# harshadms/galileo-sdr-sim

Hardware: AMD Instinct MI355X
Metric: IQ Msamples/s (×real-time @2.6MS/s), 12-SV static E1B/C, 1/2/4/8 GPU (higher is better)
Workload: dtype f64 (NCO phases) + int16x2 (packed accumulate) -> int16 IQ; 1 GPU; M-SYN12: static-geometry 12-SV E1B/C, 1199 epochs x 260000 samples @2.6 MS/s per GPU (one independent scenario per rank); channels=12, chunk_samples=1024, walk_passes=1, synth_runs_max=1, chain_mismatch=0, pipeline_depth=2, window_mode=1, kernel_family=1, output_checksum=26e91314

## Files before the change

### galileo-sdr-sim_amd/csrc/synth_group.hip

```cpp
#include <hip/hip_runtime.h>
#include <stdint.h>
#include <type_traits>

#include "nco_walk.h"
#include "synth_dev.h"
#include "synth_common.h"

using namespace galnco;
using namespace galdev;

#if !defined(GAL_GTU)
#define GAL_GTU_MAIN 1
#define GAL_GTU_WIDE 1
#define GAL_GTU_SEARCH 1
#else
#define GAL_GTU_MAIN (GAL_GTU == 0)
#define GAL_GTU_WIDE (GAL_GTU == 1)
#define GAL_GTU_SEARCH (GAL_GTU == 2)
#endif

#ifndef SG_THREADS
#define SG_THREADS 1024
#endif
#ifndef SG_WAVES_PER_EU
#define SG_WAVES_PER_EU 4
#endif
#define SG_CHUNK 1024
#define SG_SYMS 64
#define SG_STR_PITCH 580
#define SG_MPOS 17
#define SG_LUT_N 1152
#define SG_AMB 128u
#define SG_BIAS (1049088.0 + 1.4901161193847656250e-08)
#define SG_MAXCH 12
#define SG_MAXCH_WIDE 24

struct SgRec {
    double yc;
    double pm;
    double s;
    double dabs;
};
typedef uint32_t sg_u4 __attribute__((ext_vector_type(4)));
typedef const __attribute__((address_space(3))) sg_u4 *sg_lds_u4;
typedef const __attribute__((address_space(3))) int *sg_lds_int;
typedef const __attribute__((address_space(3))) uint32_t *sg_lds_u32;

__device__ __forceinline__ uint32_t sg_rep(const uint32_t w, const int d)
{
    const uint32_t lo = (uint32_t)__builtin_amdgcn_sbfe((int)w, 2 * d, 1);
    const uint32_t hi = (uint32_t)__builtin_amdgcn_sbfe((int)w, 2 * d + 1, 1);
    return gal_bfi(0x55555555u, lo, hi);
}

__device__ __forceinline__ double sg_f64(const uint32_t lo, const uint32_t hi) { return u2d(((uint64_t)hi << 32) | lo); }

template <int J0, int CNT, int MODE, int SIG, int BINS, int BPITCH, bool SEARCH>
__device__ __forceinline__ void sg_part(int (&o)[16], uint32_t &amb, uint64_t &undec, const double g16, const SgRec *rec, const uint32_t *sya,
                                        const double *s_c511, const uint32_t *s_lutd,
                                        const uint32_t *s_str, const uint2 *s_bin, const uint4 *s_pat, const uint2 *s_bin6,
                                        const uint32_t *s_pat6, const float *s_thr, const int nact)
{
    uint32_t X[CNT];
    [[maybe_unused]] uint32_t XB[CNT];
    double t[CNT];
    double c511[CNT];
    uint32_t lutd[CNT];
#pragma unroll
    for (int q = 0; q < CNT; ++q) {
        c511[q] = ((const volatile __attribute__((address_space(3))) double *)(uintptr_t)s_c511)[J0 + q];
        lutd[q] = ((const volatile __attribute__((address_space(3))) uint32_t *)(uintptr_t)s_lutd)[J0 + q];
    }
    {
        int ic0[CNT];
        float f[CNT];
        uint2 be[CNT];
        uint32_t lo[CNT], hi[CNT], mask[CNT];
        double praw[CNT];
        [[maybe_unused]] float f6[CNT];
        [[maybe_unused]] uint2 be6[CNT];
        [[maybe_unused]] int i12[CNT];
#pragma unroll
        for (int q = 0; q < CNT; ++q) {
            const int j = J0 + q;
            const sg_u4 r0 = ((sg_lds_u4)(uintptr_t)(rec + j))[0], r1 = ((sg_lds_u4)(uintptr_t)(rec + j))[1];
            const uint32_t sa0 = *(sg_lds_u32)(uintptr_t)(sya + j);
            const double A = __builtin_fma(g16, sg_f64(r1.x, r1.y), sg_f64(r0.x, r0.y));
            ic0[q] = (int)A;
            f[q] = (float)__builtin_amdgcn_fract(A);
            if constexpr (!SEARCH) {
                const int bi = (int)(f[q] * (float)BINS);
                be[q] = s_bin[j * BPITCH + bi];
            }
            if constexpr (SIG == 1) {
                const double y6 = 6.0 * A;
                i12[q] = (int)y6;
                f6[q] = (float)__builtin_amdgcn_fract(y6);
                be6[q] = s_bin6[j * CB_BIN_PITCH + (int)(f6[q] * (float)CB_BINS)];
            }
            const uint32_t *wp = s_str + j * SG_STR_PITCH + (ic0[q] >> 4);
            lo[q] = wp[0];
            hi[q] = wp[1];
            int pos;
            asm("v_med3_i32 %0, %1, 0, 16" : "=v"(pos) : "v"(ic0[q] - (8184 - 16)));
            mask[q] = *(sg_lds_u32)(uintptr_t)(sa0 + ((uint32_t)pos << 2));
            praw[q] = __builtin_fma(g16, sg_f64(r1.z, r1.w), sg_f64(r0.z, r0.w));
        }
        uint4 M[CNT];
        [[maybe_unused]] uint32_t p6[CNT];
#pragma unroll
        for (int q = 0; q < CNT; ++q) {
            const int j = J0 + q;
            if constexpr (SIG == 1) {
                const float thr6 = __uint_as_float(be6[q].x);
                const uint32_t po6 = be6[q].y + (f6[q] >= thr6 ? 4u : 0u);
                p6[q] = *reinterpret_cast<const uint32_t *>(reinterpret_cast<const char *>(s_pat6 + j * 16) + po6) ^
                        (((uint32_t)i12[q] & 1u) ? 0xAAAAAAAAu : 0u);
                undec |= __builtin_amdgcn_ballot_w64(!(__builtin_fabsf(f6[q] - thr6) >= RW_DELTA));
            }
            if constexpr (SEARCH) {
                const float *th = s_thr + j * 16;
                int id = th[7] <= f[q] ? 8 : 0;
                id += th[id + 3] <= f[q] ? 4 : 0;
                id += th[id + 1] <= f[q] ? 2 : 0;
                id += th[id] <= f[q] ? 1 : 0;
                const float up = th[id], lo = th[id > 0 ? id - 1 : 0];
                M[q] = s_pat[j * 16 + id];
                const bool near = !(up - f[q] >= RW_DELTA) | ((id > 0) & !(f[q] - lo >= RW_DELTA)) | !(f[q] >= RW_DELTA) | !(f[q] <= 1.0f - RW_DELTA);
                undec |= __builtin_amdgcn_ballot_w64(near);
            } else {
            const float thr = __uint_as_float(be[q].x);
            const uint32_t po = be[q].y + (f[q] >= thr ? 16u : 0u);
            M[q] = *reinterpret_cast<const uint4 *>(reinterpret_cast<const char *>(s_pat + j * 16) + po);
            undec |= __builtin_amdgcn_ballot_w64(!(__builtin_fabsf(f[q] - thr) >= RW_DELTA));
            }
            const double pg = praw[q] - __builtin_trunc(praw[q]);
            t[q] = __builtin_fma(511.0, pg, SG_BIAS);
        }
#pragma unroll
        for (int q = 0; q < CNT; ++q) {
            const uint32_t W = __builtin_amdgcn_alignbit(hi[q], lo[q], (uint32_t)ic0[q] << 1) ^ mask[q];
            if constexpr (SIG == 1) {
                uint32_t x, hw;
                if constexpr (MODE == 1) {
                    x = rw_spread(W, M[q]);
                    hw = ((M[q].x ^ M[q].y ^ M[q].z ^ M[q].w) & 0xAAAAAAAAu) ^ 0x22222222u;
                } else if constexpr (MODE == 4) {
                    x = gal_bfi(M[q].w, W << 16, W);
                    x = gal_bfi(M[q].z, x << 8, x);
                    x = gal_bfi(M[q].y, x << 4, x);
                    x = gal_bfi(M[q].x, x << 2, x);
                    hw = (M[q].x & 0xAAAAAAAAu) ^ 0x22222222u;
                } else {
                    x = gal_bfi(M[q].x, sg_rep(W, 1), sg_rep(W, 0));
                    x = gal_bfi(M[q].y, sg_rep(W, 2), x);
                    if constexpr (MODE == 3) {
                        x = gal_bfi(M[q].z, sg_rep(W, 3), x);
                        x = gal_bfi(M[q].w, sg_rep(W, 4), x);
                    }
                    hw = ((M[q].x ^ M[q].y ^ M[q].z ^ M[q].w) & 0xAAAAAAAAu) ^ 0xAAAAAAAAu;
                }
                hw ^= ((uint32_t)ic0[q] & 1u) ? 0xAAAAAAAAu : 0u;
                X[q] = window_signed(x);
                const uint32_t sb = x ^ hw ^ p6[q];
                const uint32_t lo1 = ~x & 0x55555555u;
                XB[q] = (J0 + q) < nact ? (lo1 | (sb & (lo1 << 1))) : 0u;
            } else if constexpr (MODE == 1) {
                X[q] = rw_spread(window_signed(W), M[q]);
            } else if constexpr (MODE == 4) {
                uint32_t x = window_signed(W);
                x = gal_bfi(M[q].w, x << 16, x);
                x = gal_bfi(M[q].z, x << 8, x);
                x = gal_bfi(M[q].y, x << 4, x);
                X[q] = gal_bfi(M[q].x, x << 2, x);
            } else {
                const uint32_t w = window_signed(W);
                uint32_t x = gal_bfi(M[q].x, sg_rep(w, 1), sg_rep(w, 0));
                x = gal_bfi(M[q].y, sg_rep(w, 2), x);
                if constexpr (MODE == 3) {
                    x = gal_bfi(M[q].z, sg_rep(w, 3), x);
                    x = gal_bfi(M[q].w, sg_rep(w, 4), x);
                }
                X[q] = x;
            }
        }
    }
    __builtin_amdgcn_sched_barrier(0);
    typedef int sg_i2 __attribute__((ext_vector_type(2)));
    typename std::conditional<SIG == 1, sg_i2, int>::type e[16][CNT];
    uint32_t lw[16][CNT];
#define SG_ISSUE(u)                                                                                                       \
    _Pragma("unroll") for (int q = 0; q < CNT; ++q) {                                                                     \
        if constexpr (SIG == 1) {                                                                                         \
            uint32_t a_;                                                                                                  \
            asm volatile("v_lshl_add_u32 %1, %2, 3, %3\n\tds_read_b64 %0, %1"                                             \
                         : "=&v"(e[u][q]), "=&v"(a_) : "v"((uint32_t)(d2u(t[q]) >> 32)), "v"(lutd[q]) : "memory");        \
        } else {                                                                                                          \
            asm volatile("v_lshl_add_u32 %0, %1, 2, %2\n\tds_read_b32 %0, %0"                                             \
                         : "=&v"(e[u][q]) : "v"((uint32_t)(d2u(t[q]) >> 32)), "v"(lutd[q]) : "memory");                   \
        }                                                                                                                 \
        lw[u][q] = (uint32_t)d2u(t[q]);                                                                                   \
        t[q] = t[q] + c511[q];                                                                                            \
    }
#define SG_WAIT(TXT, u)                                                                                                               \
    if constexpr (CNT == 1) asm volatile(TXT : "+v"(e[u][0]), "+v"(amb), "+v"(o[(u) ? (u) - 1 : 0]) :: "memory");                     \
    if constexpr (CNT == 2) asm volatile(TXT : "+v"(e[u][0]), "+v"(e[u][1]), "+v"(amb), "+v"(o[(u) ? (u) - 1 : 0]) :: "memory");      \
    if constexpr (CNT == 3) asm volatile(TXT : "+v"(e[u][0]), "+v"(e[u][1]), "+v"(e[u][2]), "+v"(amb), "+v"(o[(u) ? (u) - 1 : 0]) :: "memory"); \
    if constexpr (CNT == 4) asm volatile(TXT : "+v"(e[u][0]), "+v"(e[u][1]), "+v"(e[u][2]), "+v"(e[u][3]), "+v"(amb), "+v"(o[(u) ? (u) - 1 : 0]) :: "memory");
    SG_ISSUE(0)
#pragma unroll
    for (int u = 0; u < 16; ++u) {
        if (u < 15) {
            SG_ISSUE(u + 1)
            if constexpr (CNT == 1) { SG_WAIT("s_waitcnt lgkmcnt(1)", u) }
            if constexpr (CNT == 2) { SG_WAIT("s_waitcnt lgkmcnt(2)", u) }
            if constexpr (CNT == 3) { SG_WAIT("s_waitcnt lgkmcnt(3)", u) }
            if constexpr (CNT == 4) { SG_WAIT("s_waitcnt lgkmcnt(4)", u) }
        } else {
            SG_WAIT("s_waitcnt lgkmcnt(0)", u)
        }
        int acc = o[u];
#pragma unroll
        for (int q = 0; q < CNT; ++q) {
            if constexpr (SIG == 1) {
                gal_acc(acc, e[u][q].x, __builtin_amdgcn_sbfe((int)X[q], (uint32_t)(2 * u), 2));
                gal_acc(acc, e[u][q].y, __builtin_amdgcn_sbfe((int)XB[q], (uint32_t)(2 * u), 2));
            } else {
                gal_acc(acc, e[u][q], __builtin_amdgcn_sbfe((int)X[q], (uint32_t)(2 * u), 2));
            }
        }
#pragma unroll
        for (int q = 0; q < CNT; ++q) amb = amb < lw[u][q] ? amb : lw[u][q];
        o[u] = acc;
    }
#undef SG_WAIT
#undef SG_ISSUE
    __builtin_amdgcn_sched_barrier(0);
}

template <int NCH, bool ACC, int MODE, int SIG = 0, bool SEARCH = false>
__global__ __launch_bounds__(SG_THREADS) __attribute__((amdgpu_waves_per_eu(SG_WAVES_PER_EU)))
void k_synth_g(const DevPlan *__restrict__ Pd, SynGeom G, const uint8_t *__restrict__ act_all, const int *__restrict__ nact_all,
               uint32_t *__restrict__ iq, uint32_t *__restrict__ flist, const int flist_cap)
{
    static_assert(NCH >= 1 && NCH <= SG_MAXCH_WIDE, "1..24 channel positions per launch");
    static_assert(SIG == 0 || NCH <= SG_MAXCH, "the CBOC mode is built for up to 12 positions per launch");
    static_assert(!SEARCH || (SIG == 0 && NCH <= SG_MAXCH), "the threshold search is built for BOC(1,1), up to 12 positions per launch");
    constexpr int MC = NCH <= SG_MAXCH ? SG_MAXCH : SG_MAXCH_WIDE;
    constexpr int BINS = SIG ? CB_BINS : RW_BINS, BPITCH = SIG ? CB_BIN_PITCH : RW_BIN_PITCH;
    __shared__ uint32_t s_str[NCH * SG_STR_PITCH];
    __shared__ uint32_t s_mtab[16 * SG_MPOS];
    __shared__ __attribute__((aligned(8))) int s_lut[2 * SG_LUT_N * (SIG ? 2 : 1)];
    __shared__ uint2 s_bin[NCH * BPITCH];
    __shared__ uint4 s_pat[NCH * 16];
    __shared__ float s_thr[NCH * 16];
    __shared__ uint2 s_bin6[SIG ? NCH * CB_BIN_PITCH : 1];
    __shared__ uint32_t s_pat6[SIG ? NCH * 16 : 1];
    __shared__ float s_thr6[SIG ? NCH * 16 : 1];
    __shared__ uint32_t s_sym[NCH * SG_SYMS];
    __shared__ __attribute__((aligned(16))) SgRec s_rec[(SG_THREADS / 64) * 2 * MC];
    __shared__ double s_c511[MC];
    __shared__ uint32_t s_lutd[MC];
    __shared__ uint32_t s_sya[(SG_THREADS / 64) * 2 * MC];
    __shared__ int s_rwbad;

    const int tid = threadIdx.x;
    const int nthr = blockDim.x;
#ifdef SG_BALANCED_RANGES
    const int nb = (int)gridDim.x;
    const int xb = (nb & 7) == 0 ? (int)(blockIdx.x & 7) * (nb >> 3) + (int)(blockIdx.x >> 3) : (int)blockIdx.x;
    const long long U = (long long)G.ne * G.nchunks;
    long long uq = U * xb / nb;
    const long long u_end = U * (xb + 1) / nb;
#else
    const int bpe = G.blocks_per_epoch;
    const int er = (int)blockIdx.x / bpe, tg = (int)blockIdx.x - er * bpe;
    const int c_begin = G.nchunks * tg / bpe, c_end = G.nchunks * (tg + 1) / bpe;
#endif
    const int *const p_lut = Pd->lut;
    const int *const p_prn = Pd->prn;
    const int *const p_ib0 = Pd->ib0;
    const uint32_t *const p_str = Pd->str;
    const double *const p_cpx = Pd->cp_x, *const p_cpp = Pd->cp_p;
    const uint32_t *const p_cpi = Pd->cp_ib;
    const double *const p_cstep = Pd->cstep, *const p_dstep = Pd->dstep;
    const uint32_t *const p_pcur = Pd->page_cur, *const p_pnext = Pd->page_next;
    const uint32_t cs25 = Pd->cs25;
    int *const p_ctr = Pd->ctr;
    for (int i = tid; i < 16 * SG_MPOS; i += nthr) {
        const int pair = i / SG_MPOS, pos = i - pair * SG_MPOS;
        const uint32_t mc = (uint32_t)(pair >> 2) * 0x55555555u, mn = (uint32_t)(pair & 3) * 0x55555555u;
        s_mtab[i] = pos == 0 ? mc : pos == 16 ? mn : (mc ^ ((mc ^ mn) & (~0u << (2 * (16 - pos)))));
    }
    for (int i = tid; i < 2 * SG_LUT_N * (SIG ? 2 : 1); i += nthr) {
        if constexpr (SIG == 1) {
            const int ie = i >> 1, tab = ie >= SG_LUT_N, ii = ie - tab * SG_LUT_N;
            int k = ii < 512 ? ii - 511 : ii - 512;
            k = k >= 511 ? k - 511 : k;
            k = k >= 511 ? k - 511 : k;
            s_lut[i] = p_lut[((i & 1) << 9) + ((tab ? -k : k) & 511)];
            continue;
        }
        const int tab = i >= SG_LUT_N, ii = i - tab * SG_LUT_N;
        int k = ii < 512 ? ii - 511 : ii - 512;
        k = k >= 511 ? k - 511 : k;
        k = k >= 511 ? k - 511 : k;
        s_lut[i] = p_lut[(tab ? -k : k) & 511];
    }
#ifdef SG_BALANCED_RANGES
    int row_prn[NCH];
#pragma unroll
    for (int j = 0; j < NCH; ++j) row_prn[j] = 0;
#endif
#ifdef SG_BALANCED_RANGES
    bool first_seg = true;
    while (uq < u_end) {
    const int er = (int)(uq / G.nchunks);
    const int c_begin = (int)(uq - (long long)er * G.nchunks);
    const int c_end = (long long)(G.nchunks - c_begin) < u_end - uq ? G.nchunks : c_begin + (int)(u_end - uq);
    uq += c_end - c_begin;
    if (!first_seg) __syncthreads();
    first_seg = false;
#else
    {
#endif
    const int e = G.e0 + er;

    const int nact = __builtin_amdgcn_readfirstlane(nact_all[e]);
    const uint4 aw = *reinterpret_cast<const uint4 *>(act_all + (size_t)e * GAL_ACT_ROW);
    const uint4 aw2 = MC > 16 ? *reinterpret_cast<const uint4 *>(act_all + (size_t)e * GAL_ACT_ROW + 16) : make_uint4(0u, 0u, 0u, 0u);
    const uint32_t awv[8] = {aw.x, aw.y, aw.z, aw.w, aw2.x, aw2.y, aw2.z, aw2.w};
    int ixs[MC];
#pragma unroll
    for (int j = 0; j < MC; ++j) {
        ixs[j] = __builtin_amdgcn_readfirstlane(e * G.S + (int)((awv[j >> 2] >> (8 * (j & 3))) & 0xffu));
    }

    if (tid == 0) s_rwbad = 0;
#pragma unroll
    for (int j = 0; j < NCH; ++j) {
        int prn = __builtin_amdgcn_readfirstlane(p_prn[ixs[j]]);
        prn = prn < 1 ? 1 : prn;
        const bool on = j < nact;
#ifdef SG_BALANCED_RANGES
        const int want = on ? prn : -1;
        if (want == row_prn[j]) continue;
        row_prn[j] = want;
#endif
        const uint32_t *src = p_str + (size_t)(prn - 1) * STR_WORDS;
        for (int t = tid; t < STR_WORDS - 1; t += nthr) s_str[j * SG_STR_PITCH + t] = on ? src[t] : 0u;
        if (tid < SG_STR_PITCH - (STR_WORDS - 1)) {
            const int t = tid;
            const uint32_t w = t == 0 ? ((src[STR_WORDS - 1] & 0xffffu) | (src[0] << 16)) : ((src[t - 1] >> 16) | (src[t] << 16));
            s_str[j * SG_STR_PITCH + STR_WORDS - 1 + t] = on ? w : 0u;
        }
    }
    for (int i = tid; i < NCH * SG_SYMS; i += nthr) {
        const int j = i / SG_SYMS, k = i - j * SG_SYMS;
        int ix = 0;
#pragma unroll
        for (int q = 0; q < NCH; ++q) ix = j == q ? ixs[q] : ix;
        int ibit = p_ib0[ix] + k;
        const bool nx = ibit >= GAL_N_SYM_PAGE;
        ibit = nx ? ibit - GAL_N_SYM_PAGE : ibit;
        const uint32_t *pg = (nx ? p_pnext : p_pcur) + (size_t)ix * GAL_PAGE_WORDS;
        const uint32_t dbit = (pg[ibit >> 5] >> (ibit & 31)) & 1u;
        const uint32_t sbit = (cs25 >> (ibit % 25)) & 1u;
        const uint32_t sg = (dbit ^ sbit) | (sbit << 1);
        s_sym[i] = j < nact ? sg : 0u;
    }
    double rw_s[NCH];
#pragma unroll
    for (int j = 0; j < NCH; ++j) rw_s[j] = j < nact ? uniform_f64(2.0 * p_cstep[ixs[j]]) : 0.0;
    auto rw_step_of = [&](const int jj) {
        double v = 0.0;
#pragma unroll
        for (int j = 0; j < NCH; ++j) v = jj == j ? rw_s[j] : v;
        return v;
    };
    if (tid < MC) {
        int ix = 0;
#pragma unroll
        for (int q = 0; q < NCH; ++q) ix = tid == q ? ixs[q] : ix;
        const double d = (tid < NCH && tid < nact) ? p_dstep[ix] : 0.0;
        s_c511[tid] = 511.0 * __builtin_fabs(d);
        s_lutd[tid] = SIG ? (uint32_t)(uintptr_t)(sg_lds_int)s_lut + (((uint32_t)(d2u(d) >> 32) >> 31) ? SG_LUT_N * 8u : 0u) - (0x41300000u << 3)
                          : (uint32_t)(uintptr_t)(sg_lds_int)s_lut + (((uint32_t)(d2u(d) >> 32) >> 31) ? SG_LUT_N * 4u : 0u) - (0x41300000u << 2);
    }
    for (int t = tid; t < NCH * 16; t += nthr) {
        const int j = t >> 4, u = (t & 15) + 1;
        const double s = rw_step_of(j);
        if (u <= 15) {
            const double us = (double)u * s;
            const double T = 1.0 - (us - __builtin_floor(us));
            int rank = 0;
            for (int v = 1; v <= 15; ++v) {
                const double vs = (double)v * s;
                const double Tv = 1.0 - (vs - __builtin_floor(vs));
                rank += (Tv < T) || (Tv == T && v < u);
            }
            s_thr[j * 16 + rank] = (float)T;
        } else {
            s_thr[j * 16 + 15] = 2.0f;
        }
        if constexpr (SIG == 1) {
            const double s6 = 6.0 * s;
            if (u <= 15) {
                const double us = (double)u * s6;
                const double T = 1.0 - (us - __builtin_floor(us));
                int rank = 0;
                for (int v = 1; v <= 15; ++v) {
                    const double vs = (double)v * s6;
                    const double Tv = 1.0 - (vs - __builtin_floor(vs));
                    rank += (Tv < T) || (Tv == T && v < u);
                }
                s_thr6[j * 16 + rank] = (float)T;
            } else {
                s_thr6[j * 16 + 15] = 2.0f;
            }
        }
    }
    __syncthreads();
    auto build_bins = [&](uint2 *bins, const float *thrs, const int nbins, const int pitch, const uint32_t unit) {
        for (int t = tid; t < NCH * (nbins + 1); t += nthr) {
            const int j = t / (nbins + 1), b = t - j * (nbins + 1);
            const float lo = (float)b * (1.0f / (float)nbins) - RW_EDGE, hi = (float)(b + 1) * (1.0f / (float)nbins) + RW_EDGE;
            const float *th = thrs + j * 16;
            int idb = th[7] < lo ? 8 : 0;
            idb += th[idb + 3] < lo ? 4 : 0;
            idb += th[idb + 1] < lo ? 2 : 0;
            idb += th[idb] < lo ? 1 : 0;
            const float t0 = th[idb], t1 = idb < 15 ? th[idb + 1] : 2.0f;
            int cnt = (t0 < hi) + (t1 < hi);
            float thr = t0 < hi ? t0 : 4.0f;
            uint32_t off = (uint32_t)idb * unit;
            if (b == 0) { thr = cnt ? __builtin_nanf("") : 0.0f; off -= cnt ? 0u : unit; cnt = 0; }
            if (b == nbins - 1) { thr = cnt ? __builtin_nanf("") : 1.0f; cnt = 0; }
            if (cnt >= 2 || b == nbins) thr = __builtin_nanf("");
            if (j >= nact) { thr = 4.0f; off = 0u; }
            bins[j * pitch + b] = make_uint2(__float_as_uint(thr), off);
        }
    };
    if constexpr (!SEARCH) build_bins(s_bin, s_thr, BINS, BPITCH, 16u);
    if constexpr (SIG == 1) {
        build_bins(s_bin6, s_thr6, CB_BINS, CB_BIN_PITCH, 4u);
        for (int t = tid; t < NCH * 16; t += nthr) {
            const int j = t >> 4, id = t & 15;
            const double s6 = 6.0 * rw_step_of(j);
            const double Tlo = id ? (double)s_thr6[j * 16 + id - 1] : 0.0;
            double Thi = (double)s_thr6[j * 16 + id];
            Thi = Thi > 1.0 ? 1.0 : Thi;
            const double f = 0.5 * (Tlo + Thi);
            uint32_t w = 0u;
            for (int u = 1; u <= 15; ++u)
                if ((long long)__builtin_floor(f + (double)u * s6) & 1LL) w |= 2u << (2 * u);
            s_pat6[t] = j < nact ? w : 0u;
        }
    }
    for (int t = tid; t < NCH * 16; t += nthr) {
        const int j = t >> 4, id = t & 15;
        const double s = rw_step_of(j);
        const double Tlo = id ? (double)s_thr[j * 16 + id - 1] : 0.0;
        double Thi = (double)s_thr[j * 16 + id];
        Thi = Thi > 1.0 ? 1.0 : Thi;
        const double f = 0.5 * (Tlo + Thi);
        uint32_t m0 = 0u, m1 = 0u, m2 = 0u, m3 = 0u;
        if constexpr (MODE == 4) {
            for (int u = 0; u <= 15; ++u) {
                const int hld = u - (int)__builtin_floor(f + (double)u * s);
                int pp = u;
                m0 |= (hld & 1) ? 3u << (2 * pp) : 0u;
                pp -= hld & 1;
                m1 |= (hld & 2) ? 3u << (2 * pp) : 0u;
                pp -= hld & 2;
                m2 |= (hld & 4) ? 3u << (2 * pp) : 0u;
                pp -= hld & 4;
                m3 |= (hld & 8) ? 3u << (2 * pp) : 0u;
            }
            if (j >= nact) m0 = m1 = m2 = m3 = 0u;
        } else {
        int d = 0;
        double gp = 0.0;
        for (int u = 1; u <= 15; ++u) {
            const double g = __builtin_floor(f + (double)u * s);
            if ((MODE >= 2) ? (g != gp) : (g == gp)) {
                const uint32_t m = ~0u << (2 * u);
                m0 = d == 0 ? m : m0; m1 = d == 1 ? m : m1; m2 = d == 2 ? m : m2; m3 = d == 3 ? m : m3;
                ++d;
            }
            gp = g;
        }
        if (j >= nact) m0 = m1 = m2 = m3 = 0u;
        else if (d > (MODE == 2 ? 2 : 4)) s_rwbad = 1;
        }
        s_pat[t] = make_uint4(m0, m1, m2, m3);
    }
    __syncthreads();
    const bool rw_off = __builtin_amdgcn_readfirstlane(s_rwbad) != 0;

    const int lane = tid & 63;
    const int wv = tid >> 6;
    const int nw = nthr >> 6;
    const double g16 = (double)(16 * lane);
    const int jl = lane < NCH ? lane : NCH - 1;
    int ixl = 0;
#pragma unroll
    for (int q = 0; q < NCH; ++q) ixl = jl == q ? ixs[q] : ixl;
    const bool onl = jl < nact;
    const size_t cpl = (size_t)ixl * G.CP1;
    const double dl = onl ? p_dstep[ixl] : 0.0;
    const double sl = onl ? 2.0 * p_cstep[ixl] : 0.0, dabsl = __builtin_fabs(dl);
    const uint32_t dsgnl = (uint32_t)(d2u(dl) >> 32) & 0x80000000u;
    const uint32_t *const syml = s_sym + jl * SG_SYMS - (onl ? p_ib0[ixl] : 0);
    const uint32_t mtab0 = (uint32_t)(uintptr_t)(sg_lds_u32)s_mtab;
    SgRec *const recw = s_rec + wv * 2 * MC;
    uint32_t *const syaw = s_sya + wv * 2 * MC;
    const int cstep_w = nw;
    int c = __builtin_amdgcn_readfirstlane(c_begin + wv);
    double lx = 0.0, lp = 0.0;
    uint32_t lib = 0u;
    typedef const __attribute__((address_space(1))) double *sg_gbl_f64;
    typedef const __attribute__((address_space(1))) uint32_t *sg_gbl_u32;
    const sg_gbl_f64 g_cpx = (sg_gbl_f64)(uintptr_t)p_cpx + cpl, g_cpp = (sg_gbl_f64)(uintptr_t)p_cpp + cpl;
    const sg_gbl_u32 g_cpi = (sg_gbl_u32)(uintptr_t)p_cpi + cpl;
    auto fetch = [&](const int cc) {
        const int ce = cc < c_end ? cc : c_end - 1;
        lx = g_cpx[ce];
        lp = g_cpp[ce];
        lib = g_cpi[ce];
    };
    auto stage = [&](const int buf) {
        SgRec r;
        const bool pend = lx >= 4092.0;
        const double x = pend ? lx - 4092.0 : lx;
        r.yc = onl ? x + x : 0.5;
        r.pm = onl ? u2d(d2u(lp) ^ ((uint64_t)dsgnl << 32)) : 0.25;
        if (onl && dabsl == 0.0) {
            const int k = (int)(511.0 * r.pm);
            r.pm = ((double)(k >= 0 ? k : k - 1) + 0.5) * (1.0 / 511.0);
        }
        r.s = sl;
        r.dabs = dabsl;
        if (lane < NCH) {
            recw[buf * MC + lane] = r;
            const uint32_t ks = onl ? (lib & 0xffffu) + 500u * (lib >> 16) + (pend ? 1u : 0u) : 0u;
            const uint32_t pair = syml[ks] * 4u + syml[ks + 1];
            syaw[buf * MC + lane] = mtab0 + pair * (SG_MPOS * 4u);
        }
    };
    if (c < c_end) fetch(c);
    int buf = 0;
    for (; c < c_end; c += cstep_w, buf ^= 1) {
        stage(buf);
        fetch(c + cstep_w);
        const int n0 = c * SG_CHUNK;
        const int nsteps = G.N - n0 - 16 * lane;
        if (nsteps > 0) {
        uint32_t *out = iq + (size_t)er * G.N + n0 + 16 * lane;
        const bool vec_ok = ((((size_t)er * G.N + n0) & 3) == 0) && nsteps >= 16;
        int o[16];
        if (ACC) {
            if (vec_ok) {
#pragma unroll
                for (int q = 0; q < 4; ++q) {
                    const uint4 v = *reinterpret_cast<const uint4 *>(out + 4 * q);
                    o[4 * q] = (int)v.x; o[4 * q + 1] = (int)v.y; o[4 * q + 2] = (int)v.z; o[4 * q + 3] = (int)v.w;
                }
            } else {
#pragma unroll
                for (int u = 0; u < 16; ++u) o[u] = u < nsteps ? (int)out[u] : 0;
            }
        } else {
#pragma unroll
            for (int u = 0; u < 16; ++u) o[u] = 0;
        }
        uint32_t amb = ~0u;
        uint64_t undec = rw_off ? ~0ull : 0ull;
        const SgRec *rec = recw + buf * MC;
        const uint32_t *sya = syaw + buf * MC;
#define SG_PART(J0, CNT) sg_part<J0, CNT, MODE, SIG, BINS, BPITCH, SEARCH>(o, amb, undec, g16, rec, sya, s_c511, s_lutd, s_str, s_bin, s_pat, s_bin6, s_pat6, s_thr, nact); \
                         __builtin_amdgcn_sched_barrier(0);
        if constexpr (SIG == 1 && NCH <= 3) { SG_PART(0, NCH) }
        else if constexpr (SIG == 1 && NCH == 4) { SG_PART(0, 2) SG_PART(2, 2) }
        else if constexpr (SIG == 1 && NCH == 5) { SG_PART(0, 3) SG_PART(3, 2) }
        else if constexpr (SIG == 1 && NCH == 6) { SG_PART(0, 3) SG_PART(3, 3) }
        else if constexpr (SIG == 1 && NCH == 7) { SG_PART(0, 3) SG_PART(3, 2) SG_PART(5, 2) }
        else if constexpr (SIG == 1 && NCH == 8) { SG_PART(0, 3) SG_PART(3, 3) SG_PART(6, 2) }
        else if constexpr (SIG == 1 && NCH == 9) { SG_PART(0, 3) SG_PART(3, 3) SG_PART(6, 3) }
        else if constexpr (SIG == 1 && NCH == 10) { SG_PART(0, 3) SG_PART(3, 3) SG_PART(6, 2) SG_PART(8, 2) }
        else if constexpr (SIG == 1 && NCH == 11) { SG_PART(0, 3) SG_PART(3, 3) SG_PART(6, 3) SG_PART(9, 2) }
        else if constexpr (SIG == 1 && NCH == 12) { SG_PART(0, 3) SG_PART(3, 3) SG_PART(6, 3) SG_PART(9, 3) }
        else if constexpr (NCH <= 4) { SG_PART(0, NCH) }
        else if constexpr (NCH == 5) { SG_PART(0, 3) SG_PART(3, 2) }
        else if constexpr (NCH == 6) { SG_PART(0, 3) SG_PART(3, 3) }
        else if constexpr (NCH == 7) { SG_PART(0, 4) SG_PART(4, 3) }
        else if constexpr (NCH == 8) { SG_PART(0, 4) SG_PART(4, 4) }
        else if constexpr (NCH == 9) { SG_PART(0, 3) SG_PART(3, 3) SG_PART(6, 3) }
        else if constexpr (NCH == 10) { SG_PART(0, 4) SG_PART(4, 3) SG_PART(7, 3) }
        else if constexpr (NCH == 11) { SG_PART(0, 4) SG_PART(4, 4) SG_PART(8, 3) }
        else if constexpr (NCH == 12) { SG_PART(0, 4) SG_PART(4, 4) SG_PART(8, 4) }
        else {
            SG_PART(0, 4) SG_PART(4, 4)
            constexpr int R8 = NCH - 8;
            if constexpr (R8 == 5) { SG_PART(8, 3) SG_PART(11, 2) }
            else if constexpr (R8 == 6) { SG_PART(8, 3) SG_PART(11, 3) }
            else if constexpr (R8 == 7) { SG_PART(8, 4) SG_PART(12, 3) }
            else {
                SG_PART(8, 4)
                constexpr int R12 = NCH - 12;
                if constexpr (R12 <= 4) { SG_PART(12, R12) }
                else if constexpr (R12 == 5) { SG_PART(12, 3) SG_PART(15, 2) }
                else if constexpr (R12 == 6) { SG_PART(12, 3) SG_PART(15, 3) }
                else if constexpr (R12 == 7) { SG_PART(12, 4) SG_PART(16, 3) }
                else {
                    SG_PART(12, 4)
                    constexpr int R16 = NCH - 16;
                    if constexpr (R16 <= 4) { SG_PART(16, R16) }
                    else if constexpr (R16 == 5) { SG_PART(16, 3) SG_PART(19, 2) }
                    else if constexpr (R16 == 6) { SG_PART(16, 3) SG_PART(19, 3) }
                    else if constexpr (R16 == 7) { SG_PART(16, 4) SG_PART(20, 3) }
                    else { SG_PART(16, 4) SG_PART(20, 4) }
                }
            }
        }
#undef SG_PART
        if (vec_ok) {
#pragma unroll
            for (int q = 0; q < 4; ++q)
                *reinterpret_cast<uint4 *>(out + 4 * q) = make_uint4((uint32_t)o[4 * q], (uint32_t)o[4 * q + 1], (uint32_t)o[4 * q + 2], (uint32_t)o[4 * q + 3]);
        } else {
#pragma unroll
            for (int u = 0; u < 16; ++u)
                if (u < nsteps) out[u] = (uint32_t)o[u];
        }
        if (((undec >> lane) & 1ull) | (amb < SG_AMB)) {
            const int slot = atomicAdd(p_ctr + CTR_GFLAGS, 1);
            if (slot < flist_cap) flist[slot] = ((uint32_t)er * (uint32_t)G.nchunks + (uint32_t)c) * 64u + (uint32_t)lane;
        }
        }
    }
    }
}

#if GAL_GTU_MAIN
__global__ __launch_bounds__(256) void k_repair_g(DevPlan P, SynGeom G, uint32_t *__restrict__ iq, const uint32_t *__restrict__ flist,
                                                  const int flist_cap)
{
    __shared__ int s_lut[1024];
    const int n_raw = P.ctr[CTR_GFLAGS];
    const int n = n_raw < flist_cap ? n_raw : flist_cap;
    if (n_raw > flist_cap && blockIdx.x == 0 && threadIdx.x == 0) P.ctr[CTR_GOVER] = 1;
    const int gt = blockIdx.x * blockDim.x + threadIdx.x;
    const int r = threadIdx.x & 15;
    const int nrows = (gridDim.x * blockDim.x) >> 4;
    if (((int)blockIdx.x * (int)blockDim.x >> 4) >= n) return;
    for (int i = threadIdx.x; i < 1024; i += blockDim.x) s_lut[i] = P.lut[i];
    __syncthreads();
    for (int i = gt >> 4; i < n; i += nrows) {
        const uint32_t ent = flist[i];
        const int g = (int)(ent & 63u);
        const uint32_t ec = ent >> 6;
        const int er = (int)(ec / (uint32_t)G.nchunks), c = (int)(ec - (uint32_t)er * (uint32_t)G.nchunks);
        const int e = G.e0 + er;
        const int n0 = c * G.R + 16 * g;
        int cnt = G.N - n0;
        cnt = cnt > 16 ? 16 : cnt;
        int aI[16], aQ[16];
#pragma unroll
        for (int u = 0; u < 16; ++u) aI[u] = aQ[u] = 0;
        for (int s = r; s < G.S; s += 16) {
            const int idx = e * G.S + s;
            const int prn = P.prn[idx];
            if (prn <= 0) continue;
            const size_t cp = (size_t)idx * G.CP1 + c;
            const double cst = P.cstep[idx], d = P.dstep[idx];
            const uint32_t cib = P.cp_ib[cp];
            const CodeEnd ce = code_walk(P.cp_x[cp], (int)(cib & 0xffffu), cst, 1.0 / cst, 16 * g, 1 << 30, [](int, double, int, int) {});
            double x = ce.x;
            double p = carr_walk_track(P.cp_p[cp], d, 1.0 / __builtin_fabs(d), 16 * g, 16 * g + 1, 16 * g + 1, [](int, double) {}).p;
            {
                int nR = G.N - c * G.R;
                nR = nR > G.R ? G.R : nR;
                const int rem = nR - 16 * g;
                const CodeEnd ce2 = code_walk(ce.x, ce.ibit, cst, 1.0 / cst, rem, 1 << 30, [](int, double, int, int) {});
                const uint32_t fl_end = (cib >> 16) | (uint32_t)ce.flipped | (uint32_t)ce2.flipped;
                const double p2 = carr_walk_track(p, d, 1.0 / __builtin_fabs(d), rem, rem + 1, rem + 1, [](int, double) {}).p;
                const bool bad = d2u(ce2.x) != d2u(P.cp_x[cp + 1]) || ((uint32_t)ce2.ibit | (fl_end << 16)) != P.cp_ib[cp + 1] ||
                                 d2u(p2) != d2u(P.cp_p[cp + 1]);
                if (bad) atomicAdd(&P.ctr[CTR_MISMATCH], 1);
            }
            int ib0 = ce.ibit, fl0 = (int)(cib >> 16) | ce.flipped;
            if (x >= 4092.0) {
                x -= 4092.0;
                ib0 += 1;
                if (ib0 >= GAL_N_SYM_PAGE) {
                    ib0 = 0;
                    fl0 = 1;
                }
            }
            int ib1 = ib0 + 1, fl1 = fl0;
            if (ib1 >= GAL_N_SYM_PAGE) {
                ib1 = 0;
                fl1 = 1;
            }
            const uint32_t *pg0 = (fl0 ? P.page_next : P.page_cur) + (size_t)idx * GAL_PAGE_WORDS;
            const uint32_t *pg1 = (fl1 ? P.page_next : P.page_cur) + (size_t)idx * GAL_PAGE_WORDS;
            const uint32_t *str = P.str + (size_t)(prn - 1) * STR_WORDS;
            int wb = (int)(x * 2.0) >> 4;
            wb = wb > STR_WORDS - 1 ? STR_WORDS - 1 : wb;
            const uint32_t pw0 = pg0[ib0 >> 5], pw1 = pg1[ib1 >> 5];
            const uint32_t wa0 = str[wb], wa1 = str[wb + 1 < STR_WORDS ? wb + 1 : wb], wh0 = str[0], wh1 = str[1];
            const int db0 = (int)((pw0 >> (ib0 & 31)) & 1u), sb0 = (int)((P.cs25 >> (ib0 % 25)) & 1u);
            const int db1 = (int)((pw1 >> (ib1 & 31)) & 1u), sb1 = (int)((P.cs25 >> (ib1 % 25)) & 1u);
            bool wrapped = false;
            for (int u = 0; u < cnt; ++u) {
                if (x >= 4092.0) {
                    x -= 4092.0;
                    wrapped = true;
                }
                const int k = ((int)(511.0 * p)) & 511;
                const int icode = (int)(x * 2.0);
                const int wi = icode >> 4;
                const uint32_t w = wrapped ? (wi == 0 ? wh0 : wh1) : (wi == wb ? wa0 : wa1);
                const uint32_t fld = (w >> (2 * (icode & 15))) & 3u;
                const uint32_t cbit = (fld >> 1) ^ ((uint32_t)icode & 1u), bbit = (fld & 1u) ^ cbit;
                const int sub = (icode & 1) ? 1 : -1;
                const int E1B_chip = sub * (bbit ? -1 : 1), E1C_chip = sub * (cbit ? -1 : 1);
                const int databit = (wrapped ? db1 : db0) ? -1 : 1;
                const int secCode = (wrapped ? sb1 : sb0) ? -1 : 1;
                if (P.signal == 1) {
                    const int i12 = (int)(x * 12.0);
                    const int ab = ((icode ^ i12) & 1) ? -1 : 1;
                    const int Ba = E1B_chip * databit, Ca = E1C_chip * secCode;
                    const int ta = s_lut[k], tb = s_lut[512 + k];
                    aI[u] += ((Ba - Ca) / 2) * (int)(short)(ta & 0xffff) + ab * ((Ba + Ca) / 2) * (int)(short)(tb & 0xffff);
                    aQ[u] += ((Ba - Ca) / 2) * (int)(short)((uint32_t)ta >> 16) + ab * ((Ba + Ca) / 2) * (int)(short)((uint32_t)tb >> 16);
                } else {
                    const int v = E1B_chip * databit - E1C_chip * secCode;
                    const int ent2 = s_lut[k];
                    aI[u] += (v / 2) * (int)(short)(ent2 & 0xffff);
                    aQ[u] += (v / 2) * (int)(short)((uint32_t)ent2 >> 16);
                }
                x = x + cst;
                p = carr_step(p, d);
            }
        }
#pragma unroll
        for (int u = 0; u < 16; ++u) {
            int I = aI[u], Q = aQ[u];
#pragma unroll
            for (int m = 8; m >= 1; m >>= 1) {
                I += __shfl_xor(I, m, 16);
                Q += __shfl_xor(Q, m, 16);
            }
            if (r == u && u < cnt) iq[(size_t)er * G.N + n0 + u] = ((uint32_t)(uint16_t)(short)I) | ((uint32_t)(uint16_t)(short)Q << 16);
        }
    }
}

#endif

static int sg_grid(const DevPlan *P, int ne, int nch = 0)
{
    const long long U = (long long)ne * P->nchunks;
    const bool wide = nch > SG_MAXCH;
    const int slots = (P->gslots > 0 ? P->gslots : 512) / (wide ? 2 : 1);
#ifdef SG_BALANCED_RANGES
    if (P->grounds > 0 && U >= (long long)slots * P->grounds * 32) return slots * P->grounds;
#else
    (void)U;
#endif
    int bpe = P->gbpe > 0 ? P->gbpe : 1;
    if (P->gbpe <= 0) {
        const int nw = wide ? 16 : 8;
        bpe = (slots + ne - 1) / ne;
        const int most = P->nchunks / (2 * nw) > 1 ? P->nchunks / (2 * nw) : 1;
        bpe = bpe > most ? most : bpe;
        while ((long long)ne * bpe < 4096 && P->nchunks / (bpe * 2 * nw) >= 16) bpe *= 2;
    }
    return ne * bpe;
}
static int sg_bpe(const DevPlan *P, int ne, int nch = 0)
{
    return sg_grid(P, ne, nch) / ne;
}

extern "C" int galk_launch_synth_g_wide(const DevPlan *P, const DevPlan *Pd, int nch, int accumulate, int mode, const uint8_t *act, const int *nact,
                                        uint32_t *iq, const SynGeom *G, int grid, hipStream_t st);
extern "C" int galk_launch_synth_g_search(const DevPlan *P, const DevPlan *Pd, int nch, int accumulate, int mode, const uint8_t *act, const int *nact,
                                          uint32_t *iq, const SynGeom *G, int grid, hipStream_t st);

#if GAL_GTU_WIDE
template <bool ACC, int MODE>
static int launch_wide_t(const DevPlan *P, const DevPlan *Pd, int nch, const uint8_t *act, const int *nact, uint32_t *iq, const SynGeom &G, int ngrid,
                         hipStream_t st)
{
    const dim3 grid(ngrid), wblock(SG_THREADS);
#define GAL_WCASE(n) case n: hipLaunchKernelGGL((k_synth_g<n, ACC, MODE, 0>), grid, wblock, 0, st, Pd, G, act, nact, iq, P->gflist, P->gflist_cap); return 0;
    switch (nch) {
        GAL_WCASE(13) GAL_WCASE(14) GAL_WCASE(15) GAL_WCASE(16) GAL_WCASE(17) GAL_WCASE(18)
        GAL_WCASE(19) GAL_WCASE(20) GAL_WCASE(21) GAL_WCASE(22) GAL_WCASE(23) GAL_WCASE(24)
    default: return -1;
    }
#undef GAL_WCASE
}
extern "C" int galk_launch_synth_g_wide(const DevPlan *P, const DevPlan *Pd, int nch, int accumulate, int mode, const uint8_t *act, const int *nact,
                                        uint32_t *iq, const SynGeom *G, int grid, hipStream_t st)
{
#define GAL_MCASE(m) case m: return accumulate ? launch_wide_t<true, m>(P, Pd, nch, act, nact, iq, *G, grid, st) : launch_wide_t<false, m>(P, Pd, nch, act, nact, iq, *G, grid, st);
    switch (mode) {
        GAL_MCASE(1) GAL_MCASE(2) GAL_MCASE(3) GAL_MCASE(4)
    default: return -3;
    }
#undef GAL_MCASE
}
#endif

#if GAL_GTU_SEARCH
template <bool ACC, int MODE>
static int launch_search_t(const DevPlan *P, const DevPlan *Pd, int nch, const uint8_t *act, const int *nact, uint32_t *iq, const SynGeom &G, int ngrid,
                           hipStream_t st)
{
    const dim3 grid(ngrid), block(512);
#define GAL_SCASE(n) case n: hipLaunchKernelGGL((k_synth_g<n, ACC, MODE, 0, true>), grid, block, 0, st, Pd, G, act, nact, iq, P->gflist, P->gflist_cap); return 0;
    switch (nch) {
        GAL_SCASE(1) GAL_SCASE(2) GAL_SCASE(3) GAL_SCASE(4) GAL_SCASE(5) GAL_SCASE(6)
        GAL_SCASE(7) GAL_SCASE(8) GAL_SCASE(9) GAL_SCASE(10) GAL_SCASE(11) GAL_SCASE(12)
    default: return -1;
    }
#undef GAL_SCASE
}
extern "C" int galk_launch_synth_g_search(const DevPlan *P, const DevPlan *Pd, int nch, int accumulate, int mode, const uint8_t *act, const int *nact,
                                          uint32_t *iq, const SynGeom *G, int grid, hipStream_t st)
{
#define GAL_MCASE(m) case m: return accumulate ? launch_search_t<true, m>(P, Pd, nch, act, nact, iq, *G, grid, st) : launch_search_t<false, m>(P, Pd, nch, act, nact, iq, *G, grid, st);
    switch (mode) {
        GAL_MCASE(1) GAL_MCASE(2) GAL_MCASE(3) GAL_MCASE(4)
    default: return -3;
    }
#undef GAL_MCASE
}
#endif

#if GAL_GTU_MAIN
template <bool ACC, int MODE, int SIG>
static int launch_synth_g_t(const DevPlan *P, const DevPlan *Pd, int nch, const uint8_t *act, const int *nact, uint32_t *iq, int e0,
                            int ne, hipStream_t st, const SynGeom &G)
{
    if constexpr (SIG == 0) {
        if (P->rw_search) return galk_launch_synth_g_search(P, Pd, nch, ACC ? 1 : 0, MODE, act, nact, iq, &G, sg_grid(P, ne, nch), st);
        if (nch > SG_MAXCH) return galk_launch_synth_g_wide(P, Pd, nch, ACC ? 1 : 0, MODE, act, nact, iq, &G, sg_grid(P, ne, nch), st);
    }
#ifdef SG_FORCE_THREADS
    const dim3 grid(sg_grid(P, ne, nch)), block(SG_FORCE_THREADS);
#else
    const dim3 grid(sg_grid(P, ne, nch)), block(P->gthreads >= 64 && P->gthreads <= SG_THREADS && (P->gthreads & 63) == 0 ? P->gthreads : 512);
#endif
#define GAL_CASE(n) case n: hipLaunchKernelGGL((k_synth_g<n, ACC, MODE, SIG>), grid, block, 0, st, Pd, G, act, nact, iq, P->gflist, P->gflist_cap); break;
    switch (nch) {
        GAL_CASE(1) GAL_CASE(2) GAL_CASE(3) GAL_CASE(4) GAL_CASE(5) GAL_CASE(6)
        GAL_CASE(7) GAL_CASE(8) GAL_CASE(9) GAL_CASE(10) GAL_CASE(11) GAL_CASE(12)
    default: return -1;
    }
#undef GAL_CASE
    return 0;
}

static SynGeom sg_geom(const DevPlan *P, int e0, int ne, int nch = 0)
{
    SynGeom G;
    G.e0 = e0;
    G.ne = ne;
    G.S = P->S; G.N = P->N; G.R = P->R; G.nchunks = P->nchunks; G.CP1 = P->CP1;
    G.blocks_per_epoch = ne > 0 ? sg_bpe(P, ne, nch) : 1;
    G.cls = 1;
    G.per = P->nchunks;
    return G;
}

__global__ void k_warm_g() {}
extern "C" void galk_warm_g(hipStream_t st) { hipLaunchKernelGGL(k_warm_g, dim3(1), dim3(64), 0, st); }

extern "C" int galk_launch_synth_g(const DevPlan *P, const DevPlan *Pd, int nch, int accumulate, const uint8_t *act, const int *nact,
                                   uint32_t *iq, int e0, int ne, hipStream_t st)
{
    if (P->R != SG_CHUNK) return -2;
    const SynGeom G = sg_geom(P, e0, ne, nch);
    if (P->signal == 1) {
#define SG_MODE_CASE(m) case m: return accumulate ? launch_synth_g_t<true, m, 1>(P, Pd, nch, act, nact, iq, e0, ne, st, G) \
                                                  : launch_synth_g_t<false, m, 1>(P, Pd, nch, act, nact, iq, e0, ne, st, G);
        switch (P->rw) {
            SG_MODE_CASE(1) SG_MODE_CASE(2) SG_MODE_CASE(3) SG_MODE_CASE(4)
        default: return -3;
        }
#undef SG_MODE_CASE
    }
#define SG_MODE_CASE(m) case m: return accumulate ? launch_synth_g_t<true, m, 0>(P, Pd, nch, act, nact, iq, e0, ne, st, G) \
                                                  : launch_synth_g_t<false, m, 0>(P, Pd, nch, act, nact, iq, e0, ne, st, G);
    switch (P->rw) {
        SG_MODE_CASE(1) SG_MODE_CASE(2) SG_MODE_CASE(3) SG_MODE_CASE(4)
    default: return -3;
    }
#undef SG_MODE_CASE
}

extern "C" void galk_launch_repair_g(const DevPlan *P, uint32_t *iq, int e0, hipStream_t st)
{
    const SynGeom G = sg_geom(P, e0, 0);
    hipLaunchKernelGGL(k_repair_g, dim3(512), dim3(256), 0, st, *P, G, iq, P->gflist, P->gflist_cap);
}
#endif
```

Baseline: 303,100 Msamples/s.

## Use biased-double fixed-point bits for code phase integer, fraction and bin lookup

For the BOC(1,1) non-search path, a 2^20 bias is added to the code-phase accumulator so the double's high word holds the integer phase and its low word holds a 32-bit fixed-point fraction. This replaces the f64-to-int conversion, fract, float multiply and bin indexing with bit extraction, and the per-bin thresholds become 32-bit integers compared with a single SDWA-based subtract/select sequence. The goal is fewer VALU instructions in the hot per-channel inner loop. In exchange it relies on hand-written inline asm, a reworked bin table encoding and the bias keeping the exponent fixed, which risks subtle correctness problems at bin edges.

```diff
diff --git a/galileo-sdr-sim_amd/csrc/synth_group.hip b/galileo-sdr-sim_amd/csrc/synth_group.hip
--- a/galileo-sdr-sim_amd/csrc/synth_group.hip
+++ b/galileo-sdr-sim_amd/csrc/synth_group.hip
@@ -32,6 +32,10 @@
 #define SG_LUT_N 1152
 #define SG_AMB 128u
 #define SG_BIAS (1049088.0 + 1.4901161193847656250e-08)
+#define SG_YBIAS 1048576.0
+#define SG_YEXP 0x41300000u
+#define SG_DW 1024u
+#define SG_FIX(SIG, SEARCH) ((SIG) == 0 && !(SEARCH))
 #define SG_MAXCH 12
 #define SG_MAXCH_WIDE 24
 
@@ -73,7 +77,8 @@
     }
     {
         int ic0[CNT];
-        float f[CNT];
+        [[maybe_unused]] float f[CNT];
+        [[maybe_unused]] uint32_t fw[CNT];
         uint2 be[CNT];
         uint32_t lo[CNT], hi[CNT], mask[CNT];
         double praw[CNT];
@@ -86,9 +91,15 @@
             const sg_u4 r0 = ((sg_lds_u4)(uintptr_t)(rec + j))[0], r1 = ((sg_lds_u4)(uintptr_t)(rec + j))[1];
             const uint32_t sa0 = *(sg_lds_u32)(uintptr_t)(sya + j);
             const double A = __builtin_fma(g16, sg_f64(r1.x, r1.y), sg_f64(r0.x, r0.y));
+            if constexpr (SG_FIX(SIG, SEARCH)) {
+                ic0[q] = (int)(uint32_t)(d2u(A) >> 32);
+                fw[q] = (uint32_t)d2u(A);
+                be[q] = s_bin[j * BPITCH + (fw[q] >> (32 - __builtin_ctz(BINS)))];
+            } else {
             ic0[q] = (int)A;
             f[q] = (float)__builtin_amdgcn_fract(A);
-            if constexpr (!SEARCH) {
+            }
+            if constexpr (!SEARCH && !SG_FIX(SIG, SEARCH)) {
                 const int bi = (int)(f[q] * (float)BINS);
                 be[q] = s_bin[j * BPITCH + bi];
             }
@@ -98,11 +109,11 @@
                 f6[q] = (float)__builtin_amdgcn_fract(y6);
                 be6[q] = s_bin6[j * CB_BIN_PITCH + (int)(f6[q] * (float)CB_BINS)];
             }
-            const uint32_t *wp = s_str + j * SG_STR_PITCH + (ic0[q] >> 4);
+            const uint32_t *wp = s_str + j * SG_STR_PITCH + (SG_FIX(SIG, SEARCH) ? (int)__builtin_amdgcn_ubfe((uint32_t)ic0[q], 4, 16) : (ic0[q] >> 4));
             lo[q] = wp[0];
             hi[q] = wp[1];
             int pos;
-            asm("v_med3_i32 %0, %1, 0, 16" : "=v"(pos) : "v"(ic0[q] - (8184 - 16)));
+            asm("v_med3_i32 %0, %1, 0, 16" : "=v"(pos) : "v"(ic0[q] - (8184 - 16) - (SG_FIX(SIG, SEARCH) ? (int)SG_YEXP : 0)));
             mask[q] = *(sg_lds_u32)(uintptr_t)(sa0 + ((uint32_t)pos << 2));
             praw[q] = __builtin_fma(g16, sg_f64(r1.z, r1.w), sg_f64(r0.z, r0.w));
         }
@@ -128,6 +139,16 @@
                 M[q] = s_pat[j * 16 + id];
                 const bool near = !(up - f[q] >= RW_DELTA) | ((id > 0) & !(f[q] - lo >= RW_DELTA)) | !(f[q] >= RW_DELTA) | !(f[q] <= 1.0f - RW_DELTA);
                 undec |= __builtin_amdgcn_ballot_w64(near);
+            } else if constexpr (SG_FIX(SIG, SEARCH)) {
+                uint32_t d, po, sh;
+                asm("v_sub_co_u32 %0, vcc, %3, %4\n\t"
+                    "v_and_b32_sdwa %0, %0, sext(%5) dst_sel:DWORD dst_unused:UNUSED_PAD src0_sel:DWORD src1_sel:BYTE_2\n\t"
+                    "v_lshlrev_b32 %2, 1, %6\n\t"
+                    "v_cndmask_b32_sdwa %1, %5, %5, vcc dst_sel:DWORD dst_unused:UNUSED_PAD src0_sel:BYTE_0 src1_sel:BYTE_1"
+                    : "=&v"(d), "=&v"(po), "=&v"(sh) : "v"(be[q].x), "v"(fw[q]), "v"(be[q].y), "v"(ic0[q]) : "vcc");
+                ic0[q] = (int)sh;
+                M[q] = *reinterpret_cast<const uint4 *>(reinterpret_cast<const char *>(s_pat + j * 16) + po);
+                undec |= __builtin_amdgcn_ballot_w64(d <= 2u * SG_DW);
             } else {
             const float thr = __uint_as_float(be[q].x);
             const uint32_t po = be[q].y + (f[q] >= thr ? 16u : 0u);
@@ -139,7 +160,7 @@
         }
 #pragma unroll
         for (int q = 0; q < CNT; ++q) {
-            const uint32_t W = __builtin_amdgcn_alignbit(hi[q], lo[q], (uint32_t)ic0[q] << 1) ^ mask[q];
+            const uint32_t W = __builtin_amdgcn_alignbit(hi[q], lo[q], SG_FIX(SIG, SEARCH) ? (uint32_t)ic0[q] : (uint32_t)ic0[q] << 1) ^ mask[q];
             if constexpr (SIG == 1) {
                 uint32_t x, hw;
                 if constexpr (MODE == 1) {
@@ -246,6 +267,7 @@
     static_assert(NCH >= 1 && NCH <= SG_MAXCH_WIDE, "1..24 channel positions per launch");
     static_assert(SIG == 0 || NCH <= SG_MAXCH, "the CBOC mode is built for up to 12 positions per launch");
     static_assert(!SEARCH || (SIG == 0 && NCH <= SG_MAXCH), "the threshold search is built for BOC(1,1), up to 12 positions per launch");
+    static_assert(!SG_FIX(SIG, SEARCH) || (RW_BINS & (RW_BINS - 1)) == 0, "the fixed-point bin index is the top bits of the fraction word");
     constexpr int MC = NCH <= SG_MAXCH ? SG_MAXCH : SG_MAXCH_WIDE;
     constexpr int BINS = SIG ? CB_BINS : RW_BINS, BPITCH = SIG ? CB_BIN_PITCH : RW_BIN_PITCH;
     __shared__ uint32_t s_str[NCH * SG_STR_PITCH];
@@ -421,7 +443,7 @@
         }
     }
     __syncthreads();
-    auto build_bins = [&](uint2 *bins, const float *thrs, const int nbins, const int pitch, const uint32_t unit) {
+    auto build_bins = [&](uint2 *bins, const float *thrs, const int nbins, const int pitch, const uint32_t unit, const bool fix = false) {
         for (int t = tid; t < NCH * (nbins + 1); t += nthr) {
             const int j = t / (nbins + 1), b = t - j * (nbins + 1);
             const float lo = (float)b * (1.0f / (float)nbins) - RW_EDGE, hi = (float)(b + 1) * (1.0f / (float)nbins) + RW_EDGE;
@@ -432,6 +454,16 @@
             idb += th[idb] < lo ? 1 : 0;
             const float t0 = th[idb], t1 = idb < 15 ? th[idb + 1] : 2.0f;
             int cnt = (t0 < hi) + (t1 < hi);
+            if (fix) {
+                const bool edge = b == 0 || b == nbins - 1, has = cnt == 1 && !edge, on = j < nact;
+                const uint32_t o = on ? (uint32_t)idb * unit : 0u;
+                const uint32_t far = ((uint32_t)b << (32 - __builtin_ctz(RW_BINS))) ^ 0x80000000u;
+                const uint32_t x = !on ? far : has ? (uint32_t)(t0 * 4294967296.0f) + SG_DW
+                                   : edge ? SG_DW : far;
+                const bool und = on && (cnt >= 2 || b == nbins || (edge && cnt));
+                bins[j * pitch + b] = make_uint2(x, o | ((has && on ? o + unit : o) << 8) | (und ? 0u : 0xff0000u));
+                continue;
+            }
             float thr = t0 < hi ? t0 : 4.0f;
             uint32_t off = (uint32_t)idb * unit;
             if (b == 0) { thr = cnt ? __builtin_nanf("") : 0.0f; off -= cnt ? 0u : unit; cnt = 0; }
@@ -441,7 +473,7 @@
             bins[j * pitch + b] = make_uint2(__float_as_uint(thr), off);
         }
     };
-    if constexpr (!SEARCH) build_bins(s_bin, s_thr, BINS, BPITCH, 16u);
+    if constexpr (!SEARCH) build_bins(s_bin, s_thr, BINS, BPITCH, 16u, SG_FIX(SIG, SEARCH));
     if constexpr (SIG == 1) {
         build_bins(s_bin6, s_thr6, CB_BINS, CB_BIN_PITCH, 4u);
         for (int t = tid; t < NCH * 16; t += nthr) {
@@ -534,6 +566,7 @@
         const bool pend = lx >= 4092.0;
         const double x = pend ? lx - 4092.0 : lx;
         r.yc = onl ? x + x : 0.5;
+        if constexpr (SG_FIX(SIG, SEARCH)) r.yc += SG_YBIAS;
         r.pm = onl ? u2d(d2u(lp) ^ ((uint64_t)dsgnl << 32)) : 0.25;
         if (onl && dabsl == 0.0) {
             const int k = (int)(511.0 * r.pm);
```

Measured after the change: 308,600 Msamples/s (median of 6 runs). +1.8%, better.
